# nl1xx/simple-multimodal

Measured on AMD Instinct MI355X. Metric: fusion fwd+bwd samples/sec at B=16 d=768, higher is better.
Workload: dtype bf16

## Files before the change

include/mmfusion.h:

```cpp
#ifndef MMFUSION_H
#define MMFUSION_H

#include <stddef.h>
#include <stdint.h>

#ifdef __cplusplus
extern "C" {
#endif

#define MMF_ABI_VERSION 1

enum {
  MMF_OK = 0,
  MMF_E_SHAPE = -1,
  MMF_E_DTYPE = -2,
  MMF_E_ALIGN = -3,
  MMF_E_LAUNCH = -4,
  MMF_E_UNSUPPORTED = -5
};

int mmf_version(void);
const char* mmf_last_error(void);
int mmf_device_cu_count(void);

// ... 21 lines not shown

int mmf_gemm_grouped(const mmf_gemm_problem* problems, int num_problems, int layout,
                     int epilogue, int out_f32, void* stream);
typedef struct mmf_gemm_extra {
  float alpha;
  float dropout_p;
  const uint64_t* rng_state;
  uint32_t site;
} mmf_gemm_extra;
int mmf_gemm_grouped_ex(const mmf_gemm_problem* problems, int num_problems, int layout, int epilogue,
                        int out_f32, const mmf_gemm_extra* extra, void* stream);

int mmf_gemm_select_impl(int impl);
int mmf_gemm_last_impl(void);
int mmf_gemm_set_persistent_workgroups(int n);

#define MMF_SKINNY_MAX_PROBLEMS 24
typedef struct mmf_skinny_problem {
  const void* X;
  const void* W;
  void* Y;
  const float* bias;
  const void* aux;
  int32_t M, N, K;
  int32_t ldx, ldw, ldy, ldaux;
} mmf_skinny_problem;
int mmf_skinny_linear_fwd(const mmf_skinny_problem* problems, int num_problems, int flags, int out_f32, void* stream);
int mmf_skinny_linear_dgrad(const mmf_skinny_problem* problems, int num_problems, int flags, float alpha, int out_f32,
                            void* stream);
int mmf_skinny_last_strip(void);
// ... 212 lines not shown
```

simple-multimodal_amd/csrc/gemm7.hip:

```cpp
#include <algorithm>
#include "gemm6_parts.h"

namespace {

constexpr int BK = 32, NS = 4;
constexpr int TILE = 256 * BK * 2, STAGE = 2 * TILE, PPO = BK / 8, PPW = 2 * PPO;

typedef int i32x4_t __attribute__((ext_vector_type(4)));

struct TileSrc {
  const unsigned short* Ab;
  const unsigned short* Bb;
  int recA, recB, stepB, KT;
};
struct TileDst {
  int pi, m0, n0;
};

__device__ __forceinline__ int to_sgpr(int x) {
  int r;
  asm volatile("s_nop 0\n\tv_readfirstlane_b32 %0, %1\n\ts_nop 4" : "=s"(r) : "v"(x));
  return r;
}

template <bool B_KR>
__device__ __forceinline__ void locate_tile(const GemmArgs& args, const int total_tiles, const int orig, TileSrc& s, TileDst& d, int& lda, int& ldb) {
  const int bid = to_sgpr(mmf_xcd_tile(orig, total_tiles, args.xcd_granule));
  int pi = 0;
  while (pi + 1 < args.nprob && bid >= args.tile_start[pi + 1]) ++pi;
  const mmf_gemm_problem& P = args.p[pi];
  int m0, n0;
  tile_origin(P, bid - args.tile_start[pi], m0, n0);
  m0 = to_sgpr(m0);
  n0 = to_sgpr(n0);
  d.pi = pi; d.m0 = m0; d.n0 = n0;
  lda = P.lda; ldb = P.ldb;
  s.Ab = static_cast<const unsigned short*>(P.A) + (size_t)m0 * P.lda;
  s.Bb = static_cast<const unsigned short*>(P.B) + (B_KR ? (size_t)n0 : (size_t)n0 * P.ldb);
  s.recA = (int)(((long)(P.M - m0 - 1) * P.lda + P.K) * 2);
  s.recB = (int)((B_KR ? ((long)(P.K - 1) * P.ldb + (P.N - n0)) : ((long)(P.N - n0 - 1) * P.ldb + P.K)) * 2);
  s.stepB = (B_KR ? BK * P.ldb : BK) * 2;
  s.KT = P.K / BK;
}

template <int CT>
__device__ __forceinline__ void drain_tile(const GemmArgs& args, const int pi, const mmf_gemm_problem& P, const int mb, const int nb,
                                           f32x16_t (&acc)[4][4], char* region, const int lane) {
  constexpr bool AUX = (CT & (MMF_EPI_MASK_AUX | MMF_EPI_ADD_AUX)) != 0;
  constexpr bool DROP = (CT & MMF_EPI_DROPOUT) != 0;
  const unsigned drop_key = DROP ? mmf_rng_key(*args.rng_state, args.site, (unsigned)args.orig[pi]) : 0u;
  const float drop_scale = DROP ? 1.f / (1.f - (float)args.drop_thresh * (1.f / 4294967296.f)) : 1.f;
  const float alpha = (CT & MMF_EPI_MASK_AUX) ? args.alpha : 1.f;
  const int r = lane & 31, h = lane >> 5, q = lane >> 4, cq = lane & 15;
  const unsigned wr_base = (unsigned)(r * 256 + 8 * h + 16 * (r & 15));
  const unsigned rd_base = (unsigned)(q * 256 + ((cq ^ q) << 4));
  auto acc_at = [&](int c) { return region + (wr_base ^ (unsigned)(c << 4)); };
  auto row_at = [&](int it) { return region + it * 1024 + (rd_base ^ (unsigned)((it & 3) << 6)); };
  const bool col_ok = nb + 8 * cq < P.N;
  const __amdgpu_buffer_rsrc_t crs = __builtin_amdgcn_make_buffer_rsrc(P.C, 0, (int)((((long)P.M - 1) * P.ldc + P.N) * 2), 0x00020000);
  const __amdgpu_buffer_rsrc_t ars = __builtin_amdgcn_make_buffer_rsrc(const_cast<void*>(AUX ? P.aux : P.C), 0,
                                                                       AUX ? (int)((((long)P.M - 1) * P.ldaux + P.N) * 2) : 0, 0x00020000);
  const unsigned c_off0 = col_ok ? (unsigned)(((long)(mb + q) * P.ldc + nb + 8 * cq) * 2) : 0x80000000u;
  const unsigned a_off0 = col_ok ? (unsigned)(((long)(mb + q) * P.ldaux + nb + 8 * cq) * 2) : 0x80000000u;
  const unsigned c_row4 = (unsigned)(4 * P.ldc * 2), a_row4 = (unsigned)(4 * P.ldaux * 2);

  u32x4_t auxr[2][8];
  auto load_aux = [&](int tm, int slot) {
#pragma unroll
    for (int it = 0; it < 8; ++it)
      auxr[slot][it] = __builtin_bit_cast(u32x4_t, __builtin_amdgcn_raw_buffer_load_b128(ars, a_off0 + (unsigned)(8 * tm + it) * a_row4, 0, 0));
  };
  if constexpr (AUX) { load_aux(0, 0); load_aux(1, 1); }
#pragma unroll
  for (int tm = 0; tm < 4; ++tm) {
    u32x2_t axv[4][4];
    if constexpr (AUX) {
#pragma unroll
      for (int it = 0; it < 8; ++it) *reinterpret_cast<u32x4_t*>(row_at(it)) = auxr[tm & 1][it];
#pragma unroll
      for (int tn = 0; tn < 4; ++tn)
#pragma unroll
        for (int g = 0; g < 4; ++g) axv[tn][g] = *reinterpret_cast<const u32x2_t*>(acc_at(4 * tn + g));
      __builtin_amdgcn_sched_barrier(0);
      if (tm + 2 < 4) load_aux(tm + 2, tm & 1);
      __builtin_amdgcn_sched_barrier(0);
    }
#pragma unroll
    for (int tn = 0; tn < 4; ++tn) {
      asm volatile("" : "+a"(acc[tn][tm]));
#pragma unroll
      for (int g = 0; g < 4; ++g) {
        f32x4_t v = {acc[tn][tm][4 * g], acc[tn][tm][4 * g + 1], acc[tn][tm][4 * g + 2], acc[tn][tm][4 * g + 3]};
        if constexpr (CT & MMF_EPI_RELU) {
#pragma unroll
          for (int e = 0; e < 4; ++e) v[e] = fmaxf(v[e], 0.f);
        }
        if constexpr (DROP) {
          const unsigned idx = (unsigned)(mb + 32 * tm + r) * (unsigned)P.N + (unsigned)(nb + 32 * tn + 8 * g + 4 * h);
#pragma unroll
// ... 10 lines not shown
          }
        }
        *reinterpret_cast<u32x2_t*>(acc_at(4 * tn + g)) = u32x2_t{pack_bf16x2(v[0], v[1]), pack_bf16x2(v[2], v[3])};
      }
      __builtin_amdgcn_sched_barrier(0);
    }
    u32x4_t w[8];
#pragma unroll
    for (int it = 0; it < 8; ++it) w[it] = *reinterpret_cast<const u32x4_t*>(row_at(it));
#pragma unroll
    for (int it = 0; it < 8; ++it) __builtin_amdgcn_raw_buffer_store_b128(w[it], crs, c_off0 + (unsigned)(8 * tm + it) * c_row4, 0, 0);
    __builtin_amdgcn_sched_barrier(0);
  }
}

template <bool B_KR, int CT>
__device__ __forceinline__ void gemm7_body(const GemmArgs& args, const int total_tiles, char* smem) {
  constexpr bool A_KR = false;
  constexpr int WA = BK, WB = B_KR ? 256 : BK;

  const int tid = threadIdx.x, lane = tid & 63;
  const int wave = __builtin_amdgcn_readfirstlane(tid >> 6);
  const int wm = wave >> 1, wn = wave & 1;
  const int nwg = gridDim.x;
  const int wid = blockIdx.x;
  auto walk = [&](int round) { return round * nwg + ((round & 1) ? nwg - 1 - wid : wid); };
  int round = 0;
  int orig = walk(0);
  TileSrc ns;
  TileDst cd, nd;
  int KT, lda, ldb;
  locate_tile<B_KR>(args, total_tiles, orig, ns, cd, lda, ldb);
  KT = ns.KT;

  unsigned voff[PPW], voffn[PPW];
  auto set_voff = [&](unsigned (&v)[PPW], int la, int lb) {
#pragma unroll
    for (int i = 0; i < PPO; ++i) {
      v[i] = piece_voff<A_KR, BK>(wave + 4 * i, la, lane);
      v[PPO + i] = piece_voff<B_KR, BK>(wave + 4 * i, lb, lane);
    }
  };
  set_voff(voff, lda, ldb);
  char* const my_pieces = smem + wave * 1024;

  struct Desc { int lo, hi, rec; };
  auto mkdesc = [](const unsigned short* p, int rec) {
    const unsigned long long a = (unsigned long long)(uintptr_t)p;
    return Desc{(int)(unsigned)a, (int)((unsigned)(a >> 32) & 0xffffu), rec};
  };
  auto advance = [](Desc& d, int bytes) {
    const unsigned long long a = (((unsigned long long)(unsigned)d.hi << 32) | (unsigned)d.lo) + (unsigned long long)bytes;
    d.lo = (int)(unsigned)a; d.hi = (int)(unsigned)(a >> 32);
    int r;
    asm("s_sub_i32 %0, %1, %2\n\ts_max_i32 %0, %0, 0" : "=s"(r) : "s"(d.rec), "s"(bytes) : "scc");
    d.rec = r;
  };
  Desc dA = mkdesc(ns.Ab, ns.recA);
  Desc dB = mkdesc(ns.Bb, ns.recB);
  constexpr int stepA = BK * 2;
  int stepB = ns.stepB;
  const unsigned lds_pieces = (unsigned)(uintptr_t)(const __attribute__((address_space(3))) char*)my_pieces;
  auto hot_piece = [&](auto ic, const unsigned ring_base) {
    constexpr int I = decltype(ic)::value, OFF = I < PPO ? I * 4096 : TILE + (I - PPO) * 4096;
    const Desc& d = I < PPO ? dA : dB;
    const i32x4_t q = {d.lo, d.hi, d.rec, 0x00020000};
    asm volatile("s_add_i32 m0, %0, %3\n\ts_nop 0\n\tbuffer_load_dwordx4 %1, %2, 0 offen lds" ::"s"(ring_base), "v"(voff[I]), "s"(q), "n"(OFF) : "memory");
    __builtin_amdgcn_sched_barrier(0);
  };

#pragma unroll
  for (int s = 0; s < NS; ++s) {
    const unsigned rb = lds_pieces + (unsigned)(s * STAGE);
    hot_piece(std::integral_constant<int, 0>{}, rb); hot_piece(std::integral_constant<int, 1>{}, rb);
    hot_piece(std::integral_constant<int, 2>{}, rb); hot_piece(std::integral_constant<int, 3>{}, rb);
    if (s + 1 < NS) {
      hot_piece(std::integral_constant<int, 4>{}, rb); hot_piece(std::integral_constant<int, 5>{}, rb);
      hot_piece(std::integral_constant<int, 6>{}, rb); hot_piece(std::integral_constant<int, 7>{}, rb);
      advance(dA, stepA); advance(dB, stepB);
    }
  }

  bool has_next = walk(1) < total_tiles;
  nd = cd;
  if (has_next) {
    int la, lb;
    locate_tile<B_KR>(args, total_tiles, walk(1), ns, nd, la, lb);
    set_voff(voffn, la, lb);
  } else {
    ns.recA = 0; ns.recB = 0; ns.stepB = 0;
#pragma unroll
    for (int i = 0; i < PPW; ++i) voffn[i] = voff[i];
  }

  unsigned la0, la1, lb0, lb1;
  Frag4<A_KR>::lane_parts(WA, lane, la0, la1);
  Frag4<B_KR>::lane_parts(WB, lane, lb0, lb1);
  const unsigned smem_base = (unsigned)(uintptr_t)(const __attribute__((address_space(3))) char*)smem;
  const unsigned qa = (unsigned)((WA / 32) * 2048 * 4 * wm);
  const unsigned qb = (unsigned)(B_KR ? 512 * 4 * wn : (WB / 32) * 2048 * 4 * wn);
  la0 += smem_base + qa; la1 += smem_base + qa;
  lb0 += smem_base + TILE + qb; lb1 += smem_base + TILE + qb;

  f32x16_t acc[4][4];

  constexpr bool use_bias = (CT & MMF_EPI_BIAS) != 0;
  float bcur[4] = {0.f, 0.f, 0.f, 0.f};
  auto load_bias = [&](float (&b)[4], const TileDst& d) {
    const mmf_gemm_problem& P = args.p[d.pi];
    const __amdgpu_buffer_rsrc_t brs = __builtin_amdgcn_make_buffer_rsrc(const_cast<float*>(P.bias), 0, P.N * 4, 0x00020000);
    const unsigned off = (unsigned)((d.n0 + 128 * wn + (lane & 31)) * 4);
#pragma unroll
    for (int tn = 0; tn < 4; ++tn)
      b[tn] = __uint_as_float((unsigned)__builtin_amdgcn_raw_buffer_load_b32(brs, off + (unsigned)(32 * tn * 4), 0, 0));
  };
  auto split3 = [&](float x) {
    const bool lo = lane < 32;
    const unsigned hh = __float_as_uint(x) & 0xffff0000u;
    const float r1 = x - __uint_as_float(hh);
    const unsigned mm = __float_as_uint(r1) & 0xffff0000u;
    const float r2 = r1 - __uint_as_float(mm);
    const unsigned ll = __float_as_uint(r2) & 0xffff0000u;
    const u32x4_t w = {lo ? ((hh >> 16) | mm) : 0u, lo ? (ll >> 16) : 0u, 0u, 0u};
    return __builtin_bit_cast(bf16x8_t, w);
  };
  auto bias_init = [&](const float (&b)[4]) {
    const f32x16_t zero = {0.f, 0.f, 0.f, 0.f, 0.f, 0.f, 0.f, 0.f, 0.f, 0.f, 0.f, 0.f, 0.f, 0.f, 0.f, 0.f};
    const u32x4_t ow = {lane < 32 ? 0x3f803f80u : 0u, lane < 32 ? 0x00003f80u : 0u, 0u, 0u};
    u32x4_t ones[4] = {ow, ow, ow, ow};
#pragma unroll
    for (int tm = 0; tm < 4; ++tm) asm volatile("" : "+v"(ones[tm]));
#pragma unroll
    for (int tn = 0; tn < 4; ++tn) {
      u32x4_t bw = __builtin_bit_cast(u32x4_t, use_bias ? split3(b[tn]) : __builtin_bit_cast(bf16x8_t, u32x4_t{0u, 0u, 0u, 0u}));
      asm volatile("" : "+v"(bw));
#pragma unroll
      for (int tm = 0; tm < 4; ++tm) {
        acc[tn][tm] = __builtin_amdgcn_mfma_f32_32x32x16_bf16(__builtin_bit_cast(bf16x8_t, bw), __builtin_bit_cast(bf16x8_t, ones[tm]), zero, 0, 0, 0);
        __builtin_amdgcn_sched_barrier(0);
      }
    }
  };
  if constexpr (use_bias) load_bias(bcur, cd);

  vm_wait<PPW * (NS - 2) + 4>();
  __builtin_amdgcn_s_barrier();
  Frag4<A_KR> fa[2];
  Frag4<B_KR> fb[2];
  fa[0].template issue<WA, 0, 0>(la0, la1);
  fb[0].template issue<WB, 0, 0>(lb0, lb1);
  frag_wait(fa[0], fb[0]);

  auto mf = [&](const Frag4<A_KR>& a, const Frag4<B_KR>& b, int i) {
    const int tm = i >> 2, tn = i & 3;
    acc[tn][tm] = __builtin_amdgcn_mfma_f32_32x32x16_bf16(b.get(tn), a.get(tm), acc[tn][tm], 0, 0, 0);
    asm volatile("" ::"a"(acc[tn][tm]));
    __builtin_amdgcn_sched_barrier(0);
  };
#define MMF_G7_READ(dstA, dstB, G, u, so)                                                              \
  do {                                                                                                 \
    if ((u) == 0) dstA.template issue1<WA, G, 0, 0>(la0 + (so), la1 + (so));                            \
    if ((u) == 1) dstA.template issue1<WA, G, 0, 1>(la0 + (so), la1 + (so));                            \
    if ((u) == 2) dstA.template issue1<WA, G, 0, 2>(la0 + (so), la1 + (so));                            \
    if ((u) == 3) dstA.template issue1<WA, G, 0, 3>(la0 + (so), la1 + (so));                            \
    if ((u) == 4) dstB.template issue1<WB, G, 0, 0>(lb0 + (so), lb1 + (so));                            \
    if ((u) == 5) dstB.template issue1<WB, G, 0, 1>(lb0 + (so), lb1 + (so));                            \
    if ((u) == 6) dstB.template issue1<WB, G, 0, 2>(lb0 + (so), lb1 + (so));                            \
    if ((u) == 7) dstB.template issue1<WB, G, 0, 3>(lb0 + (so), lb1 + (so));                            \
    __builtin_amdgcn_sched_barrier(0);                                                                 \
  } while (0)

  auto stage = [&](const unsigned g, const int kt, const int ksw) {
    unsigned long long swmask;
    const Desc nA = mkdesc(ns.Ab, ns.recA), nB = mkdesc(ns.Bb, ns.recB);
    const unsigned so = (g % NS) * STAGE;
    const unsigned ring_cur = lds_pieces + so, ring_prev = lds_pieces + ((g + NS - 1) % NS) * STAGE;
#pragma unroll
    for (int i = 0; i < 16; ++i) {
      mf(fa[0], fb[0], i);
      if (i < 8) MMF_G7_READ(fa[1], fb[1], 1, i, so);
      if (i == 8)  hot_piece(std::integral_constant<int, 4>{}, ring_prev);
      if (i == 10) hot_piece(std::integral_constant<int, 5>{}, ring_prev);
      if (i == 12) hot_piece(std::integral_constant<int, 6>{}, ring_prev);
      if (i == 14) hot_piece(std::integral_constant<int, 7>{}, ring_prev);
    }
    frag_wait(fa[1], fb[1]);
    const unsigned sn = ((g + 1) % NS) * STAGE;
#pragma unroll
    for (int i = 0; i < 4; ++i) mf(fa[1], fb[1], i);
    vm_wait<PPW * (NS - 2)>();
    __builtin_amdgcn_s_barrier();
    __builtin_amdgcn_sched_barrier(0);
#pragma unroll
    for (int i = 4; i < 16; ++i) {
      mf(fa[1], fb[1], i);
      if (i < 12) MMF_G7_READ(fa[0], fb[0], 0, i - 4, sn);
      if (i == 4) {
        advance(dA, stepA);
        advance(dB, stepB);
        asm volatile("" ::"s"(dA.lo), "s"(dA.hi), "s"(dA.rec), "s"(dB.lo), "s"(dB.hi), "s"(dB.rec));
        __builtin_amdgcn_sched_barrier(0);
      }
      if (i == 5) {
        asm volatile("s_cmp_eq_u32 %8, %16\n\t"
                     "s_cselect_b32 %0, %9, %0\n\ts_cselect_b32 %1, %10, %1\n\ts_cselect_b32 %2, %11, %2\n\t"
                     "s_cselect_b32 %3, %12, %3\n\ts_cselect_b32 %4, %13, %4\n\ts_cselect_b32 %5, %14, %5\n\t"
                     "s_cselect_b32 %6, %15, %6\n\ts_cselect_b64 %7, -1, 0"
                     : "+s"(dA.lo), "+s"(dA.hi), "+s"(dA.rec), "+s"(dB.lo), "+s"(dB.hi), "+s"(dB.rec), "+s"(stepB), "=s"(swmask)
                     : "s"(kt), "s"(nA.lo), "s"(nA.hi), "s"(nA.rec), "s"(nB.lo), "s"(nB.hi), "s"(nB.rec), "s"(ns.stepB), "s"(ksw)
                     : "scc");
        __builtin_amdgcn_sched_barrier(0);
      }
      if (i == 6) {
        asm volatile("v_cndmask_b32_e64 %0, %0, %4, %8\n\tv_cndmask_b32_e64 %1, %1, %5, %8\n\t"
                     "v_cndmask_b32_e64 %2, %2, %6, %8\n\tv_cndmask_b32_e64 %3, %3, %7, %8"
                     : "+v"(voff[0]), "+v"(voff[1]), "+v"(voff[2]), "+v"(voff[3])
                     : "v"(voffn[0]), "v"(voffn[1]), "v"(voffn[2]), "v"(voffn[3]), "s"(swmask));
        __builtin_amdgcn_sched_barrier(0);
      }
      if (i == 7) {
        asm volatile("v_cndmask_b32_e64 %0, %0, %4, %8\n\tv_cndmask_b32_e64 %1, %1, %5, %8\n\t"
                     "v_cndmask_b32_e64 %2, %2, %6, %8\n\tv_cndmask_b32_e64 %3, %3, %7, %8"
                     : "+v"(voff[4]), "+v"(voff[5]), "+v"(voff[6]), "+v"(voff[7])
                     : "v"(voffn[4]), "v"(voffn[5]), "v"(voffn[6]), "v"(voffn[7]), "s"(swmask));
        __builtin_amdgcn_sched_barrier(0);
      }
      if (i == 12) hot_piece(std::integral_constant<int, 0>{}, ring_cur);
      if (i == 13) hot_piece(std::integral_constant<int, 1>{}, ring_cur);
      if (i == 14) hot_piece(std::integral_constant<int, 2>{}, ring_cur);
      if (i == 15) hot_piece(std::integral_constant<int, 3>{}, ring_cur);
    }
    frag_wait(fa[0], fb[0]);
  };

  char* const region = smem + NS * STAGE + wave * 8192;
  unsigned g = 0;
  for (;;) {
    bias_init(bcur);
    const int ksw = KT - NS;
    for (int kt = 0; kt < KT; ++kt, ++g) stage(g, kt, ksw);
    const mmf_gemm_problem& P = args.p[cd.pi];
    const int mb = cd.m0 + 128 * wm, nb = cd.n0 + 128 * wn;
    if constexpr (use_bias) { if (has_next) load_bias(bcur, nd); }
#ifndef MMF_G7_NODRAIN
    drain_tile<CT & ~MMF_EPI_BIAS>(args, cd.pi, P, mb, nb, acc, region, lane);
#else
    if (lane == 0 && mb == -1) static_cast<volatile unsigned short*>(P.C)[0] = (unsigned short)acc[0][0][0];
#endif
    if (!has_next) break;
    ++round;
    orig = walk(round);
    cd = nd;
    KT = ns.KT;
    has_next = walk(round + 1) < total_tiles;
    if (has_next) {
      int la, lb;
      locate_tile<B_KR>(args, total_tiles, walk(round + 1), ns, nd, la, lb);
      set_voff(voffn, la, lb);
    } else {
      ns.recA = 0; ns.recB = 0; ns.stepB = 0;
    }
  }
  vm_wait<0>();
#undef MMF_G7_READ
}

template <bool B_KR, int CT>
__global__ __launch_bounds__(NTHREADS, 1)
void gemm7_persistent_kernel(const GemmArgs args, const int total_tiles) {
  __shared__ __attribute__((aligned(1024))) char smem[NS * STAGE + 4 * 8192];
  gemm7_body<B_KR, CT>(args, total_tiles, smem);
}

template <bool B_KR, int CT>
void launch7(const GemmArgs& a, int total, int grid, hipStream_t s) {
  hipLaunchKernelGGL((gemm7_persistent_kernel<B_KR, CT>), dim3(grid), dim3(NTHREADS), 0, s, a, total);
}
bool launch7_select(int layout, int eflags, const GemmArgs* a, int total, int grid, hipStream_t s) {
  if (layout == MMF_GEMM_NT) {
    if (eflags == 0)                                      { if (a) launch7<false, 0>(*a, total, grid, s); return true; }
    if (eflags == MMF_EPI_BIAS)                           { if (a) launch7<false, MMF_EPI_BIAS>(*a, total, grid, s); return true; }
    if (eflags == (MMF_EPI_BIAS | MMF_EPI_RELU))          { if (a) launch7<false, MMF_EPI_BIAS | MMF_EPI_RELU>(*a, total, grid, s); return true; }
    if (eflags == (MMF_EPI_BIAS | MMF_EPI_ADD_AUX))       { if (a) launch7<false, MMF_EPI_BIAS | MMF_EPI_ADD_AUX>(*a, total, grid, s); return true; }
    if (eflags == (MMF_EPI_BIAS | MMF_EPI_RELU | MMF_EPI_DROPOUT)) {
      if (a) launch7<false, MMF_EPI_BIAS | MMF_EPI_RELU | MMF_EPI_DROPOUT>(*a, total, grid, s);
      return true;
    }
  } else if (layout == MMF_GEMM_NN) {
    if (eflags == 0)                                      { if (a) launch7<true, 0>(*a, total, grid, s); return true; }
    if (eflags == MMF_EPI_MASK_AUX)                       { if (a) launch7<true, MMF_EPI_MASK_AUX>(*a, total, grid, s); return true; }
    if (eflags == MMF_EPI_ADD_AUX)                        { if (a) launch7<true, MMF_EPI_ADD_AUX>(*a, total, grid, s); return true; }
  }
  return false;
}
}

static int g_persistent_wgs = [] { const char* e = getenv("MMF_GEMM7_WGS"); const int v = e ? atoi(e) : 0; return v > 0 ? v : 0; }();
extern "C" int mmf_gemm_set_persistent_workgroups(int n) {
  if (n < 0 || n > 65536) MMF_FAIL(MMF_E_SHAPE, "mmf_gemm_set_persistent_workgroups: %d not in 0..65536", n);
  g_persistent_wgs = n;
  return MMF_OK;
}

bool mmf_gemm7_supports(const mmf_gemm_problem* problems, int num_problems, int layout, int epilogue, int out_f32, const mmf_gemm_extra* extra) {
  if (out_f32 || !launch7_select(layout, epilogue, nullptr, 0, 0, nullptr)) return false;
  if (extra && extra->alpha != 1.f && !(layout == MMF_GEMM_NN && epilogue == MMF_EPI_MASK_AUX)) return false;
  if ((epilogue & MMF_EPI_DROPOUT) && !(extra && extra->rng_state)) return false;
  for (int i = 0; i < num_problems; ++i) {
    const mmf_gemm_problem& p = problems[i];
    if (p.K % BK || p.K < (NS + 1) * BK || (p.N & 7) || (p.ldc & 7) || (p.aux && (p.ldaux & 7))) return false;
  }
  return true;
}

int mmf_gemm7_launch(const mmf_gemm_problem* problems, int num_problems, int layout, int epilogue,
                     int out_f32, const mmf_gemm_extra* extra, hipStream_t s) {
  if (!mmf_gemm7_supports(problems, num_problems, layout, epilogue, out_f32, extra))
    MMF_FAIL(MMF_E_UNSUPPORTED, "mmf_gemm_grouped: the persistent kernel takes NT / NN launches with bf16 output, K %% 32 == 0, K >= %d, N and the "
             "leading dimensions of C / aux multiples of 8, and the flag sets of the fusion step (alpha only with the NN ReLU mask)", (NS + 1) * BK);
  GemmArgs a;
// ... 11 lines not shown
  for (int i = 0; i < num_problems; ++i) {
    const mmf_gemm_problem& p = problems[order[i]];
    const size_t a_bytes = (size_t)p.M * p.lda * 2;
    const size_t b_bytes = (size_t)(layout == MMF_GEMM_NT ? p.N : p.K) * p.ldb * 2;
    const size_t c_bytes = (size_t)p.M * p.ldc * 2, x_bytes = p.aux ? (size_t)p.M * p.ldaux * 2 : 0;
    if (a_bytes >= 0x7fffffffull || b_bytes >= 0x7fffffffull || c_bytes >= 0x7fffffffull || x_bytes >= 0x7fffffffull)
      MMF_FAIL(MMF_E_UNSUPPORTED, "mmf_gemm_grouped[%d]: operand larger than 2 GiB", i);
    a.tile_start[i] = total;
    total += ((p.M + BM - 1) / BM) * ((p.N + BN - 1) / BN);
    a.p[i] = p;
    a.orig[i] = (short)order[i];
  }
  a.tile_start[num_problems] = total;
  static const int cus = [] { int c = mmf_device_cu_count(); return c > 0 ? c : 256; }();
  const int want = g_persistent_wgs > 0 ? g_persistent_wgs : cus;
  const int grid = total < want ? total : want;
  launch7_select(layout, epilogue, &a, total, grid, s);
  MMF_CHECK_LAUNCH("mmf_gemm_grouped(v7)");
  return MMF_OK;
}
```

simple-multimodal_amd/csrc/mmf_internal.h:

```cpp
#pragma once
#include <hip/hip_runtime.h>
#include <stdint.h>
#include <stdio.h>
#include <stdlib.h>
#include <stdarg.h>
#include "../../include/mmfusion.h"

typedef __attribute__((ext_vector_type(8))) __bf16 bf16x8_t;
typedef __attribute__((ext_vector_type(4))) short s16x4_t;
typedef __attribute__((ext_vector_type(8))) short s16x8_t;
typedef __attribute__((ext_vector_type(4))) float f32x4_t;
typedef __attribute__((ext_vector_type(16))) float f32x16_t;
typedef __attribute__((ext_vector_type(4))) unsigned u32x4_t;
typedef __attribute__((ext_vector_type(2))) unsigned u32x2_t;

#define MMF_WAVE 64

void mmf_set_error(const char* fmt, ...);
#define MMF_FAIL(code, ...) do { mmf_set_error(__VA_ARGS__); return (code); } while (0)
#define MMF_CHECK_LAUNCH(name) do { hipError_t e_ = hipGetLastError(); \
  if (e_ != hipSuccess) MMF_FAIL(MMF_E_LAUNCH, "%s: launch failed: %s", name, hipGetErrorString(e_)); } while (0)

static inline bool mmf_aligned16(const void* p) { return (reinterpret_cast<uintptr_t>(p) & 15u) == 0; }

// ... 13 lines not shown
}
__device__ __forceinline__ float bf16lo(unsigned w) { return __uint_as_float(w << 16); }
__device__ __forceinline__ float bf16hi(unsigned w) { return __uint_as_float(w & 0xffff0000u); }

__device__ __forceinline__ float wave_sum(float v) {
#pragma unroll
  for (int o = 32; o > 0; o >>= 1) v += __shfl_xor(v, o, 64);
  return v;
}
__device__ __forceinline__ float wave_max(float v) {
#pragma unroll
  for (int o = 32; o > 0; o >>= 1) v = fmaxf(v, __shfl_xor(v, o, 64));
  return v;
}

__device__ __forceinline__ int mmf_xcd_tile(int orig, int total, int G) {
  const int xcd = orig & 7;
  const int full = G > 0 ? (total / (8 * G)) * (8 * G) : 0;
  if (orig < full) {
    const int j = orig >> 3;
    return ((j / G) * 8 + xcd) * G + (j % G);
  }
  const int rest = total - full, q = rest >> 3, r = rest & 7;
  return full + (xcd < r ? xcd * (q + 1) : r * (q + 1) + (xcd - r) * q) + ((orig - full) >> 3);
}
static inline int mmf_xcd_granule() {
  static const int g = [] { const char* e = getenv("MMF_GEMM_XCD_GRANULE"); const int v = e ? atoi(e) : 32; return v > 0 ? v : 0; }();
  return g;
}

__device__ __forceinline__ unsigned mmf_mix32(unsigned x) {
// ... 19 lines not shown
```

simple-multimodal_amd/mmfusion/lib.py:

```python
from __future__ import annotations

import ctypes as C
import os
from typing import List, Optional, Sequence

_HERE = os.path.dirname(os.path.abspath(__file__))
LIB_PATH = os.environ.get("MMF_LIB_PATH") or os.path.join(_HERE, "libmmfusion.so")

GEMM_NT, GEMM_NN, GEMM_TN = 0, 1, 2
EPI_BIAS, EPI_RELU, EPI_MASK_AUX, EPI_ADD_AUX, EPI_ACCUM, EPI_COLSUM_A, EPI_DROPOUT = 1, 2, 4, 8, 16, 32, 64
GEMM_MAX_PROBLEMS, ATTN_MAX_PROBLEMS, LN_MAX_PROBLEMS, COLSUM_MAX_PROBLEMS = 48, 12, 8, 24
EVAL_MAX_HEADS, EVAL_NSUMS = 4, 4

SYMBOLS = (
    "mmf_version", "mmf_last_error", "mmf_device_cu_count", "mmf_gemm_grouped", "mmf_gemm_grouped_ex", "mmf_gemm_select_impl", "mmf_gemm_last_impl", "mmf_gemm_set_persistent_workgroups",
    "mmf_attn_fwd_grouped_ex", "mmf_attn_bwd_grouped_ex", "mmf_dropout", "mmf_attn_select_impl",
    "mmf_attn_fwd_grouped", "mmf_attn_bwd_grouped", "mmf_layernorm_fwd_grouped",
    "mmf_layernorm_bwd_grouped", "mmf_layernorm_bwd_workspace_bytes", "mmf_layernorm_last_form", "mmf_cast_f32_to_bf16", "mmf_cast_bf16_to_f32", "mmf_cast_bf16_to_f32_scaled", "mmf_cast_f32_to_bf16_2d", "mmf_add3_bf16", "mmf_add3_grouped", "mmf_addn_bf16", "mmf_addn_grouped",
    "mmf_meanpool_fwd", "mmf_meanpool_bwd", "mmf_meanpool_cat_fwd", "mmf_meanpool_cat_bwd", "mmf_colsum_bf16", "mmf_colsum_grouped", "mmf_relu_bwd_bf16", "mmf_relu_bwd_mixed",
    "mmf_sqnorm_f32", "mmf_adamw_step", "mmf_adamw_advance", "mmf_skinny_linear_fwd", "mmf_skinny_linear_dgrad", "mmf_skinny_linear_fwd_ex", "mmf_skinny_linear_dgrad_ex", "mmf_skinny_last_strip",
    "mmf_gat3_dense_fwd", "mmf_gat3_dense_bwd", "mmf_infonce_fwd", "mmf_infonce_bwd", "mmf_adaptive_combine_fwd",
    "mmf_adaptive_combine_bwd", "mmf_adaptive_attn_weights", "mmf_linear_narrow_fwd", "mmf_linear_narrow_bwd", "mmf_stack3_embed_fwd",
    "mmf_stack3_embed_bwd", "mmf_rowmask_apply", "mmf_zero_ranges_f32", "mmf_fusion_loss", "mmf_modality_dropout",
    "mmf_attn_weights_mean", "mmf_gemm_f32_grouped", "mmf_gemm_f32_batched", "mmf_softmax_rows_f32", "mmf_softmax_bwd_rows_f32",
    "mmf_layernorm_f32_fwd", "mmf_layernorm_f32_bwd", "mmf_bilstm_workspace_bytes", "mmf_bilstm_layer_fwd", "mmf_bilstm_layer_bwd", "mmf_swap01",
    "mmf_distill_kl", "mmf_fusion_loss_kd", "mmf_robust_head_fwd", "mmf_robust_head_bwd",
    "mmf_fewshot_proto_fwd", "mmf_fewshot_proto_bwd", "mmf_fewshot_dist_fwd", "mmf_fewshot_dist_bwd",
    "mmf_eval_accumulate",
)

# ... 81 lines not shown
        raise RuntimeError(
            f"{LIB_PATH} is missing: the MI355X fusion path has no fallback. Build it with "
            f"`python -c 'import __graft_entry__ as g; g.build()'` or `make -C simple-multimodal_amd/csrc`.")
    import torch
    lib = C.CDLL(LIB_PATH)
    lib.mmf_last_error.restype = C.c_char_p
    lib.mmf_version.restype = C.c_int
    vp, i32, i64, f32 = C.c_void_p, C.c_int, C.c_int64, C.c_float
    lib.mmf_gemm_grouped.argtypes = [C.POINTER(GemmProblem), i32, i32, i32, i32, vp]
    lib.mmf_gemm_grouped_ex.argtypes = [C.POINTER(GemmProblem), i32, i32, i32, i32, C.POINTER(GemmExtra), vp]
    lib.mmf_attn_fwd_grouped_ex.argtypes = [C.POINTER(AttnProblem), i32, i32, f32, f32, vp, C.c_uint32, vp]
    lib.mmf_attn_bwd_grouped_ex.argtypes = [C.POINTER(AttnProblem), i32, i32, f32, f32, vp, C.c_uint32, vp]
    lib.mmf_dropout.argtypes = [vp, vp, i64, i32, f32, vp, C.c_uint32, vp]
    lib.mmf_attn_fwd_grouped.argtypes = [C.POINTER(AttnProblem), i32, i32, f32, vp]
    lib.mmf_attn_select_impl.argtypes = [i32]
    lib.mmf_attn_bwd_grouped.argtypes = [C.POINTER(AttnProblem), i32, i32, f32, vp]
    lib.mmf_layernorm_fwd_grouped.argtypes = [C.POINTER(LnProblem), i32, i32, f32, vp]
    lib.mmf_layernorm_bwd_grouped.argtypes = [C.POINTER(LnProblem), i32, i32, vp, C.c_size_t, vp]
    lib.mmf_layernorm_bwd_workspace_bytes.argtypes = [i32]
    lib.mmf_layernorm_bwd_workspace_bytes.restype = C.c_size_t
    lib.mmf_cast_f32_to_bf16.argtypes = [vp, vp, i64, vp]
    lib.mmf_cast_bf16_to_f32.argtypes = [vp, vp, i64, vp]
    lib.mmf_cast_bf16_to_f32_scaled.argtypes = [vp, vp, i64, f32, vp]
    lib.mmf_cast_f32_to_bf16_2d.argtypes = [vp, vp, i32, i32, i32, vp]
    lib.mmf_add3_bf16.argtypes = [vp, vp, vp, vp, i64, vp]
    lib.mmf_add3_grouped.argtypes = [C.POINTER(Add3Problem), i32, vp]
    lib.mmf_addn_bf16.argtypes = [C.POINTER(C.c_void_p), i32, vp, i64, i32, vp]
    lib.mmf_addn_grouped.argtypes = [C.POINTER(AddNProblem), i32, vp]
    lib.mmf_meanpool_fwd.argtypes = [vp, vp, i32, i32, i32, i32, vp]
    lib.mmf_meanpool_bwd.argtypes = [vp, vp, i32, i32, i32, i32, vp]
# ... 173 lines not shown
```

Measured before the change: 7309.

## Split the GEMM tail wave into half-height tiles via a second launch

Adds a half-M tile variant of the persistent gemm7 kernel, with a deeper ring to fit the freed LDS, and a host-side cost model that simulates the per-workgroup stage load. When the last partial wave of tiles would leave many CUs idle, the tail tiles are relaunched as twice as many half-height tiles, which shortens the critical path. The cost is an extra kernel launch, lower MFMA reuse per half tile, and a host-side walk over all tiles on each call. It is enabled by default (mode 1, heuristic).

Result: faster. 7389 (median of 6 runs) (+1.1%).

```diff
diff --git a/include/mmfusion.h b/include/mmfusion.h
--- a/include/mmfusion.h
+++ b/include/mmfusion.h
@@ -59,6 +59,7 @@
 int mmf_gemm_select_impl(int impl);
 int mmf_gemm_last_impl(void);
 int mmf_gemm_set_persistent_workgroups(int n);
+int mmf_gemm7_set_tail_split(int mode);
 
 #define MMF_SKINNY_MAX_PROBLEMS 24
 typedef struct mmf_skinny_problem {
diff --git a/simple-multimodal_amd/csrc/gemm7.hip b/simple-multimodal_amd/csrc/gemm7.hip
--- a/simple-multimodal_amd/csrc/gemm7.hip
+++ b/simple-multimodal_amd/csrc/gemm7.hip
@@ -1,10 +1,12 @@
 #include <algorithm>
+#include <vector>
 #include "gemm6_parts.h"
 
 namespace {
 
 constexpr int BK = 32, NS = 4;
-constexpr int TILE = 256 * BK * 2, STAGE = 2 * TILE, PPO = BK / 8, PPW = 2 * PPO;
+constexpr int ring_stages(int tm) { return tm == 256 ? NS : NS + 1; }
+constexpr int TILE = 256 * BK * 2, STAGE = 2 * TILE, PPO = BK / 8;
 
 typedef int i32x4_t __attribute__((ext_vector_type(4)));
 
@@ -23,29 +25,32 @@
   return r;
 }
 
-template <bool B_KR>
-__device__ __forceinline__ void locate_tile(const GemmArgs& args, const int total_tiles, const int orig, TileSrc& s, TileDst& d, int& lda, int& ldb) {
-  const int bid = to_sgpr(mmf_xcd_tile(orig, total_tiles, args.xcd_granule));
+template <bool B_KR, int TM>
+__device__ __forceinline__ void locate_tile(const GemmArgs& args, const int total_tiles, const int tile_base, const int orig, TileSrc& s,
+                                            TileDst& d, int& lda, int& ldb) {
+  const int id = to_sgpr(mmf_xcd_tile(orig, total_tiles, args.xcd_granule));
+  const int bid = TM == BM ? id : tile_base + (id >> 1);
   int pi = 0;
   while (pi + 1 < args.nprob && bid >= args.tile_start[pi + 1]) ++pi;
   const mmf_gemm_problem& P = args.p[pi];
   int m0, n0;
   tile_origin(P, bid - args.tile_start[pi], m0, n0);
+  if (TM != BM) m0 += (id & 1) * TM;
   m0 = to_sgpr(m0);
   n0 = to_sgpr(n0);
   d.pi = pi; d.m0 = m0; d.n0 = n0;
   lda = P.lda; ldb = P.ldb;
   s.Ab = static_cast<const unsigned short*>(P.A) + (size_t)m0 * P.lda;
   s.Bb = static_cast<const unsigned short*>(P.B) + (B_KR ? (size_t)n0 : (size_t)n0 * P.ldb);
-  s.recA = (int)(((long)(P.M - m0 - 1) * P.lda + P.K) * 2);
+  s.recA = (TM == BM || m0 < P.M) ? (int)(((long)(P.M - m0 - 1) * P.lda + P.K) * 2) : 0;
   s.recB = (int)((B_KR ? ((long)(P.K - 1) * P.ldb + (P.N - n0)) : ((long)(P.N - n0 - 1) * P.ldb + P.K)) * 2);
   s.stepB = (B_KR ? BK * P.ldb : BK) * 2;
   s.KT = P.K / BK;
 }
 
-template <int CT>
+template <int CT, int NTM>
 __device__ __forceinline__ void drain_tile(const GemmArgs& args, const int pi, const mmf_gemm_problem& P, const int mb, const int nb,
-                                           f32x16_t (&acc)[4][4], char* region, const int lane) {
+                                           f32x16_t (&acc)[4][NTM], char* region, const int lane) {
   constexpr bool AUX = (CT & (MMF_EPI_MASK_AUX | MMF_EPI_ADD_AUX)) != 0;
   constexpr bool DROP = (CT & MMF_EPI_DROPOUT) != 0;
   const unsigned drop_key = DROP ? mmf_rng_key(*args.rng_state, args.site, (unsigned)args.orig[pi]) : 0u;
@@ -72,7 +77,7 @@
   };
   if constexpr (AUX) { load_aux(0, 0); load_aux(1, 1); }
 #pragma unroll
-  for (int tm = 0; tm < 4; ++tm) {
+  for (int tm = 0; tm < NTM; ++tm) {
     u32x2_t axv[4][4];
     if constexpr (AUX) {
 #pragma unroll
@@ -82,7 +87,7 @@
 #pragma unroll
         for (int g = 0; g < 4; ++g) axv[tn][g] = *reinterpret_cast<const u32x2_t*>(acc_at(4 * tn + g));
       __builtin_amdgcn_sched_barrier(0);
-      if (tm + 2 < 4) load_aux(tm + 2, tm & 1);
+      if (tm + 2 < NTM) load_aux(tm + 2, tm & 1);
       __builtin_amdgcn_sched_barrier(0);
     }
 #pragma unroll
@@ -123,10 +128,12 @@
   }
 }
 
-template <bool B_KR, int CT>
-__device__ __forceinline__ void gemm7_body(const GemmArgs& args, const int total_tiles, char* smem) {
+template <bool B_KR, int CT, int TM>
+__device__ __forceinline__ void gemm7_body(const GemmArgs& args, const int total_tiles, const int tile_base, char* smem) {
   constexpr bool A_KR = false;
   constexpr int WA = BK, WB = B_KR ? 256 : BK;
+  constexpr int NFA = TM / 64, PA = TM / 64, PW = PA + PPO, NMF = 4 * NFA;
+  constexpr int TILE_A = TM * BK * 2, STAGE_T = TILE_A + TILE, NR = ring_stages(TM);
 
   const int tid = threadIdx.x, lane = tid & 63;
   const int wave = __builtin_amdgcn_readfirstlane(tid >> 6);
@@ -139,16 +146,15 @@
   TileSrc ns;
   TileDst cd, nd;
   int KT, lda, ldb;
-  locate_tile<B_KR>(args, total_tiles, orig, ns, cd, lda, ldb);
+  locate_tile<B_KR, TM>(args, total_tiles, tile_base, orig, ns, cd, lda, ldb);
   KT = ns.KT;
 
-  unsigned voff[PPW], voffn[PPW];
-  auto set_voff = [&](unsigned (&v)[PPW], int la, int lb) {
-#pragma unroll
-    for (int i = 0; i < PPO; ++i) {
-      v[i] = piece_voff<A_KR, BK>(wave + 4 * i, la, lane);
-      v[PPO + i] = piece_voff<B_KR, BK>(wave + 4 * i, lb, lane);
-    }
+  unsigned voff[PW], voffn[PW];
+  auto set_voff = [&](unsigned (&v)[PW], int la, int lb) {
+#pragma unroll
+    for (int i = 0; i < PA; ++i) v[i] = piece_voff<A_KR, BK>(wave + 4 * i, la, lane);
+#pragma unroll
+    for (int i = 0; i < PPO; ++i) v[PA + i] = piece_voff<B_KR, BK>(wave + 4 * i, lb, lane);
   };
   set_voff(voff, lda, ldb);
   char* const my_pieces = smem + wave * 1024;
@@ -171,21 +177,28 @@
   int stepB = ns.stepB;
   const unsigned lds_pieces = (unsigned)(uintptr_t)(const __attribute__((address_space(3))) char*)my_pieces;
   auto hot_piece = [&](auto ic, const unsigned ring_base) {
-    constexpr int I = decltype(ic)::value, OFF = I < PPO ? I * 4096 : TILE + (I - PPO) * 4096;
-    const Desc& d = I < PPO ? dA : dB;
+    constexpr int I = decltype(ic)::value, OFF = I < PA ? I * 4096 : TILE_A + (I - PA) * 4096;
+    const Desc& d = I < PA ? dA : dB;
     const i32x4_t q = {d.lo, d.hi, d.rec, 0x00020000};
     asm volatile("s_add_i32 m0, %0, %3\n\ts_nop 0\n\tbuffer_load_dwordx4 %1, %2, 0 offen lds" ::"s"(ring_base), "v"(voff[I]), "s"(q), "n"(OFF) : "memory");
     __builtin_amdgcn_sched_barrier(0);
   };
-
-#pragma unroll
-  for (int s = 0; s < NS; ++s) {
-    const unsigned rb = lds_pieces + (unsigned)(s * STAGE);
-    hot_piece(std::integral_constant<int, 0>{}, rb); hot_piece(std::integral_constant<int, 1>{}, rb);
-    hot_piece(std::integral_constant<int, 2>{}, rb); hot_piece(std::integral_constant<int, 3>{}, rb);
-    if (s + 1 < NS) {
-      hot_piece(std::integral_constant<int, 4>{}, rb); hot_piece(std::integral_constant<int, 5>{}, rb);
-      hot_piece(std::integral_constant<int, 6>{}, rb); hot_piece(std::integral_constant<int, 7>{}, rb);
+  using P0 = std::integral_constant<int, 0>;
+  using P1 = std::integral_constant<int, 1>;
+  using P2 = std::integral_constant<int, 2>;
+  using P3 = std::integral_constant<int, 3>;
+  using B0 = std::integral_constant<int, PA>;
+  using B1 = std::integral_constant<int, PA + 1>;
+  using B2 = std::integral_constant<int, PA + 2>;
+  using B3 = std::integral_constant<int, PA + 3>;
+
+#pragma unroll
+  for (int s = 0; s < NR; ++s) {
+    const unsigned rb = lds_pieces + (unsigned)(s * STAGE_T);
+    hot_piece(P0{}, rb); hot_piece(P1{}, rb);
+    if constexpr (PA > 2) { hot_piece(P2{}, rb); hot_piece(P3{}, rb); }
+    if (s + 1 < NR) {
+      hot_piece(B0{}, rb); hot_piece(B1{}, rb); hot_piece(B2{}, rb); hot_piece(B3{}, rb);
       advance(dA, stepA); advance(dB, stepB);
     }
   }
@@ -194,24 +207,24 @@
   nd = cd;
   if (has_next) {
     int la, lb;
-    locate_tile<B_KR>(args, total_tiles, walk(1), ns, nd, la, lb);
+    locate_tile<B_KR, TM>(args, total_tiles, tile_base, walk(1), ns, nd, la, lb);
     set_voff(voffn, la, lb);
   } else {
     ns.recA = 0; ns.recB = 0; ns.stepB = 0;
 #pragma unroll
-    for (int i = 0; i < PPW; ++i) voffn[i] = voff[i];
+    for (int i = 0; i < PW; ++i) voffn[i] = voff[i];
   }
 
   unsigned la0, la1, lb0, lb1;
   Frag4<A_KR>::lane_parts(WA, lane, la0, la1);
   Frag4<B_KR>::lane_parts(WB, lane, lb0, lb1);
   const unsigned smem_base = (unsigned)(uintptr_t)(const __attribute__((address_space(3))) char*)smem;
-  const unsigned qa = (unsigned)((WA / 32) * 2048 * 4 * wm);
+  const unsigned qa = (unsigned)((WA / 32) * 2048 * NFA * wm);
   const unsigned qb = (unsigned)(B_KR ? 512 * 4 * wn : (WB / 32) * 2048 * 4 * wn);
   la0 += smem_base + qa; la1 += smem_base + qa;
-  lb0 += smem_base + TILE + qb; lb1 += smem_base + TILE + qb;
-
-  f32x16_t acc[4][4];
+  lb0 += smem_base + TILE_A + qb; lb1 += smem_base + TILE_A + qb;
+
+  f32x16_t acc[4][NFA];
 
   constexpr bool use_bias = (CT & MMF_EPI_BIAS) != 0;
   float bcur[4] = {0.f, 0.f, 0.f, 0.f};
@@ -236,15 +249,15 @@
   auto bias_init = [&](const float (&b)[4]) {
     const f32x16_t zero = {0.f, 0.f, 0.f, 0.f, 0.f, 0.f, 0.f, 0.f, 0.f, 0.f, 0.f, 0.f, 0.f, 0.f, 0.f, 0.f};
     const u32x4_t ow = {lane < 32 ? 0x3f803f80u : 0u, lane < 32 ? 0x00003f80u : 0u, 0u, 0u};
-    u32x4_t ones[4] = {ow, ow, ow, ow};
-#pragma unroll
-    for (int tm = 0; tm < 4; ++tm) asm volatile("" : "+v"(ones[tm]));
+    u32x4_t ones[NFA];
+#pragma unroll
+    for (int tm = 0; tm < NFA; ++tm) { ones[tm] = ow; asm volatile("" : "+v"(ones[tm])); }
 #pragma unroll
     for (int tn = 0; tn < 4; ++tn) {
       u32x4_t bw = __builtin_bit_cast(u32x4_t, use_bias ? split3(b[tn]) : __builtin_bit_cast(bf16x8_t, u32x4_t{0u, 0u, 0u, 0u}));
       asm volatile("" : "+v"(bw));
 #pragma unroll
-      for (int tm = 0; tm < 4; ++tm) {
+      for (int tm = 0; tm < NFA; ++tm) {
         acc[tn][tm] = __builtin_amdgcn_mfma_f32_32x32x16_bf16(__builtin_bit_cast(bf16x8_t, bw), __builtin_bit_cast(bf16x8_t, ones[tm]), zero, 0, 0, 0);
         __builtin_amdgcn_sched_barrier(0);
       }
@@ -252,10 +265,14 @@
   };
   if constexpr (use_bias) load_bias(bcur, cd);
 
-  vm_wait<PPW * (NS - 2) + 4>();
+  vm_wait<PW * (NR - 2) + PA>();
   __builtin_amdgcn_s_barrier();
   Frag4<A_KR> fa[2];
   Frag4<B_KR> fb[2];
+  if constexpr (NFA < 4) {
+#pragma unroll
+    for (int k = 0; k < 2; ++k) fa[k].v[2] = fa[k].v[3] = u32x4_t{0u, 0u, 0u, 0u};
+  }
   fa[0].template issue<WA, 0, 0>(la0, la1);
   fb[0].template issue<WB, 0, 0>(lb0, lb1);
   frag_wait(fa[0], fb[0]);
@@ -270,47 +287,48 @@
   do {                                                                                                 \
     if ((u) == 0) dstA.template issue1<WA, G, 0, 0>(la0 + (so), la1 + (so));                            \
     if ((u) == 1) dstA.template issue1<WA, G, 0, 1>(la0 + (so), la1 + (so));                            \
-    if ((u) == 2) dstA.template issue1<WA, G, 0, 2>(la0 + (so), la1 + (so));                            \
-    if ((u) == 3) dstA.template issue1<WA, G, 0, 3>(la0 + (so), la1 + (so));                            \
-    if ((u) == 4) dstB.template issue1<WB, G, 0, 0>(lb0 + (so), lb1 + (so));                            \
-    if ((u) == 5) dstB.template issue1<WB, G, 0, 1>(lb0 + (so), lb1 + (so));                            \
-    if ((u) == 6) dstB.template issue1<WB, G, 0, 2>(lb0 + (so), lb1 + (so));                            \
-    if ((u) == 7) dstB.template issue1<WB, G, 0, 3>(lb0 + (so), lb1 + (so));                            \
+    if (NFA > 2 && (u) == 2) dstA.template issue1<WA, G, 0, 2>(la0 + (so), la1 + (so));                 \
+    if (NFA > 2 && (u) == 3) dstA.template issue1<WA, G, 0, 3>(la0 + (so), la1 + (so));                 \
+    if ((u) == NFA + 0) dstB.template issue1<WB, G, 0, 0>(lb0 + (so), lb1 + (so));                      \
+    if ((u) == NFA + 1) dstB.template issue1<WB, G, 0, 1>(lb0 + (so), lb1 + (so));                      \
+    if ((u) == NFA + 2) dstB.template issue1<WB, G, 0, 2>(lb0 + (so), lb1 + (so));                      \
+    if ((u) == NFA + 3) dstB.template issue1<WB, G, 0, 3>(lb0 + (so), lb1 + (so));                      \
     __builtin_amdgcn_sched_barrier(0);                                                                 \
   } while (0)
 
+  constexpr int E0 = TM == BM ? 8 : 1, HO = NMF / 4;
   auto stage = [&](const unsigned g, const int kt, const int ksw) {
     unsigned long long swmask;
     const Desc nA = mkdesc(ns.Ab, ns.recA), nB = mkdesc(ns.Bb, ns.recB);
-    const unsigned so = (g % NS) * STAGE;
-    const unsigned ring_cur = lds_pieces + so, ring_prev = lds_pieces + ((g + NS - 1) % NS) * STAGE;
-#pragma unroll
-    for (int i = 0; i < 16; ++i) {
+    const unsigned so = (g % NR) * STAGE_T;
+    const unsigned ring_cur = lds_pieces + so, ring_prev = lds_pieces + ((g + NR - 1) % NR) * STAGE_T;
+#pragma unroll
+    for (int i = 0; i < NMF; ++i) {
       mf(fa[0], fb[0], i);
-      if (i < 8) MMF_G7_READ(fa[1], fb[1], 1, i, so);
-      if (i == 8)  hot_piece(std::integral_constant<int, 4>{}, ring_prev);
-      if (i == 10) hot_piece(std::integral_constant<int, 5>{}, ring_prev);
-      if (i == 12) hot_piece(std::integral_constant<int, 6>{}, ring_prev);
-      if (i == 14) hot_piece(std::integral_constant<int, 7>{}, ring_prev);
+      if (i < NFA + 4) MMF_G7_READ(fa[1], fb[1], 1, i, so);
+      if (i == E0)     hot_piece(B0{}, ring_prev);
+      if (i == E0 + 2) hot_piece(B1{}, ring_prev);
+      if (i == E0 + 4) hot_piece(B2{}, ring_prev);
+      if (i == E0 + 6) hot_piece(B3{}, ring_prev);
     }
     frag_wait(fa[1], fb[1]);
-    const unsigned sn = ((g + 1) % NS) * STAGE;
-#pragma unroll
-    for (int i = 0; i < 4; ++i) mf(fa[1], fb[1], i);
-    vm_wait<PPW * (NS - 2)>();
+    const unsigned sn = ((g + 1) % NR) * STAGE_T;
+#pragma unroll
+    for (int i = 0; i < HO; ++i) mf(fa[1], fb[1], i);
+    vm_wait<PW * (NR - 2)>();
     __builtin_amdgcn_s_barrier();
     __builtin_amdgcn_sched_barrier(0);
 #pragma unroll
-    for (int i = 4; i < 16; ++i) {
+    for (int i = HO; i < NMF; ++i) {
       mf(fa[1], fb[1], i);
-      if (i < 12) MMF_G7_READ(fa[0], fb[0], 0, i - 4, sn);
-      if (i == 4) {
+      if (i - HO < NFA + 4) MMF_G7_READ(fa[0], fb[0], 0, i - HO, sn);
+      if (i == HO) {
         advance(dA, stepA);
         advance(dB, stepB);
         asm volatile("" ::"s"(dA.lo), "s"(dA.hi), "s"(dA.rec), "s"(dB.lo), "s"(dB.hi), "s"(dB.rec));
         __builtin_amdgcn_sched_barrier(0);
       }
-      if (i == 5) {
+      if (i == HO + 1) {
         asm volatile("s_cmp_eq_u32 %8, %16\n\t"
                      "s_cselect_b32 %0, %9, %0\n\ts_cselect_b32 %1, %10, %1\n\ts_cselect_b32 %2, %11, %2\n\t"
                      "s_cselect_b32 %3, %12, %3\n\ts_cselect_b32 %4, %13, %4\n\ts_cselect_b32 %5, %14, %5\n\t"
@@ -320,39 +338,48 @@
                      : "scc");
         __builtin_amdgcn_sched_barrier(0);
       }
-      if (i == 6) {
+      if (i == HO + 2) {
         asm volatile("v_cndmask_b32_e64 %0, %0, %4, %8\n\tv_cndmask_b32_e64 %1, %1, %5, %8\n\t"
                      "v_cndmask_b32_e64 %2, %2, %6, %8\n\tv_cndmask_b32_e64 %3, %3, %7, %8"
                      : "+v"(voff[0]), "+v"(voff[1]), "+v"(voff[2]), "+v"(voff[3])
                      : "v"(voffn[0]), "v"(voffn[1]), "v"(voffn[2]), "v"(voffn[3]), "s"(swmask));
         __builtin_amdgcn_sched_barrier(0);
       }
-      if (i == 7) {
-        asm volatile("v_cndmask_b32_e64 %0, %0, %4, %8\n\tv_cndmask_b32_e64 %1, %1, %5, %8\n\t"
-                     "v_cndmask_b32_e64 %2, %2, %6, %8\n\tv_cndmask_b32_e64 %3, %3, %7, %8"
-                     : "+v"(voff[4]), "+v"(voff[5]), "+v"(voff[6]), "+v"(voff[7])
-                     : "v"(voffn[4]), "v"(voffn[5]), "v"(voffn[6]), "v"(voffn[7]), "s"(swmask));
+      if (i == HO + 3) {
+        if constexpr (PW == 8) {
+          asm volatile("v_cndmask_b32_e64 %0, %0, %4, %8\n\tv_cndmask_b32_e64 %1, %1, %5, %8\n\t"
+                       "v_cndmask_b32_e64 %2, %2, %6, %8\n\tv_cndmask_b32_e64 %3, %3, %7, %8"
+                       : "+v"(voff[4]), "+v"(voff[5]), "+v"(voff[6]), "+v"(voff[7])
+                       : "v"(voffn[4]), "v"(voffn[5]), "v"(voffn[6]), "v"(voffn[7]), "s"(swmask));
+        } else {
+          static_assert(PW == 6, "a half tile has two A pieces and four B pieces per wave");
+          asm volatile("v_cndmask_b32_e64 %0, %0, %2, %4\n\tv_cndmask_b32_e64 %1, %1, %3, %4"
+                       : "+v"(voff[4]), "+v"(voff[5])
+                       : "v"(voffn[4]), "v"(voffn[5]), "s"(swmask));
+        }
         __builtin_amdgcn_sched_barrier(0);
       }
-      if (i == 12) hot_piece(std::integral_constant<int, 0>{}, ring_cur);
-      if (i == 13) hot_piece(std::integral_constant<int, 1>{}, ring_cur);
-      if (i == 14) hot_piece(std::integral_constant<int, 2>{}, ring_cur);
-      if (i == 15) hot_piece(std::integral_constant<int, 3>{}, ring_cur);
+      if (i == NMF - PA)     hot_piece(P0{}, ring_cur);
+      if (i == NMF - PA + 1) hot_piece(P1{}, ring_cur);
+      if constexpr (PA > 2) {
+        if (i == NMF - PA + 2) hot_piece(P2{}, ring_cur);
+        if (i == NMF - PA + 3) hot_piece(P3{}, ring_cur);
+      }
     }
     frag_wait(fa[0], fb[0]);
   };
 
-  char* const region = smem + NS * STAGE + wave * 8192;
+  char* const region = smem + NR * STAGE_T + wave * 8192;
   unsigned g = 0;
   for (;;) {
     bias_init(bcur);
-    const int ksw = KT - NS;
+    const int ksw = KT - NR;
     for (int kt = 0; kt < KT; ++kt, ++g) stage(g, kt, ksw);
     const mmf_gemm_problem& P = args.p[cd.pi];
-    const int mb = cd.m0 + 128 * wm, nb = cd.n0 + 128 * wn;
+    const int mb = cd.m0 + (TM / 2) * wm, nb = cd.n0 + 128 * wn;
     if constexpr (use_bias) { if (has_next) load_bias(bcur, nd); }
 #ifndef MMF_G7_NODRAIN
-    drain_tile<CT & ~MMF_EPI_BIAS>(args, cd.pi, P, mb, nb, acc, region, lane);
+    drain_tile<CT & ~MMF_EPI_BIAS, NFA>(args, cd.pi, P, mb, nb, acc, region, lane);
 #else
     if (lane == 0 && mb == -1) static_cast<volatile unsigned short*>(P.C)[0] = (unsigned short)acc[0][0][0];
 #endif
@@ -364,7 +391,7 @@
     has_next = walk(round + 1) < total_tiles;
     if (has_next) {
       int la, lb;
-      locate_tile<B_KR>(args, total_tiles, walk(round + 1), ns, nd, la, lb);
+      locate_tile<B_KR, TM>(args, total_tiles, tile_base, walk(round + 1), ns, nd, la, lb);
       set_voff(voffn, la, lb);
     } else {
       ns.recA = 0; ns.recB = 0; ns.stepB = 0;
@@ -378,29 +405,55 @@
 __global__ __launch_bounds__(NTHREADS, 1)
 void gemm7_persistent_kernel(const GemmArgs args, const int total_tiles) {
   __shared__ __attribute__((aligned(1024))) char smem[NS * STAGE + 4 * 8192];
-  gemm7_body<B_KR, CT>(args, total_tiles, smem);
+  gemm7_body<B_KR, CT, BM>(args, total_tiles, 0, smem);
 }
 
 template <bool B_KR, int CT>
-void launch7(const GemmArgs& a, int total, int grid, hipStream_t s) {
-  hipLaunchKernelGGL((gemm7_persistent_kernel<B_KR, CT>), dim3(grid), dim3(NTHREADS), 0, s, a, total);
-}
-bool launch7_select(int layout, int eflags, const GemmArgs* a, int total, int grid, hipStream_t s) {
+__global__ __launch_bounds__(NTHREADS, 1)
+void gemm7_half_kernel(const GemmArgs args, const int total_tiles, const int tile_base) {
+  __shared__ __attribute__((aligned(1024))) char smem[ring_stages(BM / 2) * (STAGE - TILE / 2) + 4 * 8192];
+  gemm7_body<B_KR, CT, BM / 2>(args, total_tiles, tile_base, smem);
+}
+
+template <bool B_KR, int CT>
+void launch7(const GemmArgs& a, int total, int grid, int half_base, hipStream_t s) {
+  if (half_base < 0)
+    hipLaunchKernelGGL((gemm7_persistent_kernel<B_KR, CT>), dim3(grid), dim3(NTHREADS), 0, s, a, total);
+  else
+    hipLaunchKernelGGL((gemm7_half_kernel<B_KR, CT>), dim3(grid), dim3(NTHREADS), 0, s, a, total, half_base);
+}
+bool launch7_select(int layout, int eflags, const GemmArgs* a, int total, int grid, int hb, hipStream_t s) {
   if (layout == MMF_GEMM_NT) {
-    if (eflags == 0)                                      { if (a) launch7<false, 0>(*a, total, grid, s); return true; }
-    if (eflags == MMF_EPI_BIAS)                           { if (a) launch7<false, MMF_EPI_BIAS>(*a, total, grid, s); return true; }
-    if (eflags == (MMF_EPI_BIAS | MMF_EPI_RELU))          { if (a) launch7<false, MMF_EPI_BIAS | MMF_EPI_RELU>(*a, total, grid, s); return true; }
-    if (eflags == (MMF_EPI_BIAS | MMF_EPI_ADD_AUX))       { if (a) launch7<false, MMF_EPI_BIAS | MMF_EPI_ADD_AUX>(*a, total, grid, s); return true; }
+    if (eflags == 0)                                      { if (a) launch7<false, 0>(*a, total, grid, hb, s); return true; }
+    if (eflags == MMF_EPI_BIAS)                           { if (a) launch7<false, MMF_EPI_BIAS>(*a, total, grid, hb, s); return true; }
+    if (eflags == (MMF_EPI_BIAS | MMF_EPI_RELU))          { if (a) launch7<false, MMF_EPI_BIAS | MMF_EPI_RELU>(*a, total, grid, hb, s); return true; }
+    if (eflags == (MMF_EPI_BIAS | MMF_EPI_ADD_AUX))       { if (a) launch7<false, MMF_EPI_BIAS | MMF_EPI_ADD_AUX>(*a, total, grid, hb, s); return true; }
     if (eflags == (MMF_EPI_BIAS | MMF_EPI_RELU | MMF_EPI_DROPOUT)) {
-      if (a) launch7<false, MMF_EPI_BIAS | MMF_EPI_RELU | MMF_EPI_DROPOUT>(*a, total, grid, s);
+      if (a) launch7<false, MMF_EPI_BIAS | MMF_EPI_RELU | MMF_EPI_DROPOUT>(*a, total, grid, hb, s);
       return true;
     }
   } else if (layout == MMF_GEMM_NN) {
-    if (eflags == 0)                                      { if (a) launch7<true, 0>(*a, total, grid, s); return true; }
-    if (eflags == MMF_EPI_MASK_AUX)                       { if (a) launch7<true, MMF_EPI_MASK_AUX>(*a, total, grid, s); return true; }
-    if (eflags == MMF_EPI_ADD_AUX)                        { if (a) launch7<true, MMF_EPI_ADD_AUX>(*a, total, grid, s); return true; }
+    if (eflags == 0)                                      { if (a) launch7<true, 0>(*a, total, grid, hb, s); return true; }
+    if (eflags == MMF_EPI_MASK_AUX)                       { if (a) launch7<true, MMF_EPI_MASK_AUX>(*a, total, grid, hb, s); return true; }
+    if (eflags == MMF_EPI_ADD_AUX)                        { if (a) launch7<true, MMF_EPI_ADD_AUX>(*a, total, grid, hb, s); return true; }
   }
   return false;
+}
+
+constexpr float TILE_EXTRA = 4.f, HALF = 0.8f, LAUNCH_EXTRA = 8.f;
+
+int problem_of(const GemmArgs& a, int tile) {
+  return (int)(std::upper_bound(a.tile_start + 1, a.tile_start + a.nprob, tile) - (a.tile_start + 1));
+}
+float walk_stages(const GemmArgs& a, int total, int grid) {
+  static thread_local std::vector<float> wg;
+  wg.assign(grid, 0.f);
+  for (int orig = 0; orig < total; ++orig) {
+    const int round = orig / grid, pos = orig % grid;
+    const int t = mmf_xcd_tile(orig, total, a.xcd_granule);
+    wg[(round & 1) ? grid - 1 - pos : pos] += (float)(a.p[problem_of(a, t)].K / BK) + TILE_EXTRA;
+  }
+  return *std::max_element(wg.begin(), wg.end());
 }
 }
 
@@ -411,8 +464,26 @@
   return MMF_OK;
 }
 
+static int g_tail_split = 1;
+extern "C" int mmf_gemm7_set_tail_split(int mode) {
+  if (mode < 0 || mode > 2) MMF_FAIL(MMF_E_SHAPE, "mmf_gemm7_set_tail_split: %d not in 0..2", mode);
+  g_tail_split = mode;
+  return MMF_OK;
+}
+
+static int tail_split_base(const GemmArgs& a, int total, int want) {
+  const int rounds = total / want, rest = total % want, base = rounds * want;
+  if (g_tail_split == 0 || rest == 0 || a.p[a.nprob - 1].K < (ring_stages(BM / 2) + 1) * BK) return -1;
+  if (g_tail_split == 2) return base;
+  if (2 * rest > want) return -1;
+  const float today = walk_stages(a, total, std::min(total, want));
+  const float head = rounds > 0 ? walk_stages(a, base, want) : 0.f;
+  const float split = head + LAUNCH_EXTRA + HALF * ((float)(a.p[problem_of(a, base)].K / BK) + TILE_EXTRA);
+  return split < today ? base : -1;
+}
+
 bool mmf_gemm7_supports(const mmf_gemm_problem* problems, int num_problems, int layout, int epilogue, int out_f32, const mmf_gemm_extra* extra) {
-  if (out_f32 || !launch7_select(layout, epilogue, nullptr, 0, 0, nullptr)) return false;
+  if (out_f32 || !launch7_select(layout, epilogue, nullptr, 0, 0, -1, nullptr)) return false;
   if (extra && extra->alpha != 1.f && !(layout == MMF_GEMM_NN && epilogue == MMF_EPI_MASK_AUX)) return false;
   if ((epilogue & MMF_EPI_DROPOUT) && !(extra && extra->rng_state)) return false;
   for (int i = 0; i < num_problems; ++i) {
@@ -454,8 +525,14 @@
   a.tile_start[num_problems] = total;
   static const int cus = [] { int c = mmf_device_cu_count(); return c > 0 ? c : 256; }();
   const int want = g_persistent_wgs > 0 ? g_persistent_wgs : cus;
-  const int grid = total < want ? total : want;
-  launch7_select(layout, epilogue, &a, total, grid, s);
+  const int base = tail_split_base(a, total, want);
+  if (base < 0) {
+    launch7_select(layout, epilogue, &a, total, std::min(total, want), -1, s);
+  } else {
+    if (base > 0) launch7_select(layout, epilogue, &a, base, want, -1, s);
+    const int halves = 2 * (total - base);
+    launch7_select(layout, epilogue, &a, halves, std::min(halves, want), base, s);
+  }
   MMF_CHECK_LAUNCH("mmf_gemm_grouped(v7)");
   return MMF_OK;
 }
diff --git a/simple-multimodal_amd/csrc/mmf_internal.h b/simple-multimodal_amd/csrc/mmf_internal.h
--- a/simple-multimodal_amd/csrc/mmf_internal.h
+++ b/simple-multimodal_amd/csrc/mmf_internal.h
@@ -51,7 +51,7 @@
   return v;
 }
 
-__device__ __forceinline__ int mmf_xcd_tile(int orig, int total, int G) {
+__host__ __device__ __forceinline__ int mmf_xcd_tile(int orig, int total, int G) {
   const int xcd = orig & 7;
   const int full = G > 0 ? (total / (8 * G)) * (8 * G) : 0;
   if (orig < full) {
diff --git a/simple-multimodal_amd/mmfusion/lib.py b/simple-multimodal_amd/mmfusion/lib.py
--- a/simple-multimodal_amd/mmfusion/lib.py
+++ b/simple-multimodal_amd/mmfusion/lib.py
@@ -14,6 +14,7 @@
 
 SYMBOLS = (
     "mmf_version", "mmf_last_error", "mmf_device_cu_count", "mmf_gemm_grouped", "mmf_gemm_grouped_ex", "mmf_gemm_select_impl", "mmf_gemm_last_impl", "mmf_gemm_set_persistent_workgroups",
+    "mmf_gemm7_set_tail_split",
     "mmf_attn_fwd_grouped_ex", "mmf_attn_bwd_grouped_ex", "mmf_dropout", "mmf_attn_select_impl",
     "mmf_attn_fwd_grouped", "mmf_attn_bwd_grouped", "mmf_layernorm_fwd_grouped",
     "mmf_layernorm_bwd_grouped", "mmf_layernorm_bwd_workspace_bytes", "mmf_layernorm_last_form", "mmf_cast_f32_to_bf16", "mmf_cast_bf16_to_f32", "mmf_cast_bf16_to_f32_scaled", "mmf_cast_f32_to_bf16_2d", "mmf_add3_bf16", "mmf_add3_grouped", "mmf_addn_bf16", "mmf_addn_grouped",
@@ -125,6 +126,7 @@
     lib.mmf_dropout.argtypes = [vp, vp, i64, i32, f32, vp, C.c_uint32, vp]
     lib.mmf_attn_fwd_grouped.argtypes = [C.POINTER(AttnProblem), i32, i32, f32, vp]
     lib.mmf_attn_select_impl.argtypes = [i32]
+    lib.mmf_gemm7_set_tail_split.argtypes = [i32]
     lib.mmf_attn_bwd_grouped.argtypes = [C.POINTER(AttnProblem), i32, i32, f32, vp]
     lib.mmf_layernorm_fwd_grouped.argtypes = [C.POINTER(LnProblem), i32, i32, f32, vp]
     lib.mmf_layernorm_bwd_grouped.argtypes = [C.POINTER(LnProblem), i32, i32, vp, C.c_size_t, vp]
```
